# CSB5/XNA_Basecaller

Hardware: AMD Instinct MI355X
Metric: raw signal samples/sec basecalled, chunksize 10k (higher is better)
Workload: dtype f32 (feed-forward projections split-f16x3 MFMA, recurrent projections f16 MFMA + FP8 block-scaled correction MFMA, f32 accumulate; CRF decode f32)

## Files before the change

xna_basecaller_amd/csrc/xb_api.hip:

```cpp
#include <hip/hip_runtime.h>

#include <algorithm>
#include <cmath>
#include <cstdarg>
#include <cstdio>
#include <cstdlib>
#include <cstring>
#include <map>
#include <string>
#include <vector>

#include "../../include/xna_basecaller.h"
#include "xb_internal.h"

using xb::half_t;

namespace {

thread_local std::string g_create_error;

struct DevBuf {
    void *p = nullptr;
    size_t bytes = 0;
};
// ... 2230 lines not shown
    float *d_sig = reinterpret_cast<float *>(base);
    double *d_lev = reinterpret_cast<double *>(base + b_sig);
    double *d_win = reinterpret_cast<double *>(base + b_sig + b_lev), *d_cost = d_win + b_f64 / 8;
    int32_t *d_bp = reinterpret_cast<int32_t *>(base + b_sig + b_lev + 2 * b_f64);
    int8_t *d_ok = reinterpret_cast<int8_t *>(d_bp) + b_bp;
    XB_HIP(ctx, hipMemcpyAsync(d_sig, signal, C * N * 4, hipMemcpyHostToDevice, ctx->stream));
    XB_HIP(ctx, hipMemcpyAsync(d_lev, levels, total * 8, hipMemcpyHostToDevice, ctx->stream));
    if (band) XB_HIP(ctx, hipMemcpyAsync(d_win, window, C * 8, hipMemcpyHostToDevice, ctx->stream));
    if (int rc = dtw_run(ctx, d_sig, n, N, d_lev, offsets, ref_rep, d_win, band, Kmax, {d_bp, d_ok, d_cost})) return rc;
    XB_HIP(ctx, hipMemcpyAsync(breakpoints, d_bp, C * Kmax * 4, hipMemcpyDeviceToHost, ctx->stream));
    XB_HIP(ctx, hipMemcpyAsync(ok, d_ok, C, hipMemcpyDeviceToHost, ctx->stream));
    XB_HIP(ctx, hipMemcpyAsync(cost, d_cost, C * 8, hipMemcpyDeviceToHost, ctx->stream));
    return xb_synchronize(ctx);
}

XB_API int64_t xb_dtw_scratch_bytes(const xb_ctx *ctx) { return ctx ? (int64_t)ctx->dtw.scratch_written : 0; }

XB_API int xb_set_profiling(xb_ctx *ctx, int on)
{
    if (!ctx) return XB_ERR_INVALID;
    XB_HIP(ctx, hipSetDevice(ctx->device));
    if (int rc = flush_held(ctx)) return rc;
    ctx->profiling = on != 0;
    return XB_OK;
}

XB_API int xb_get_stage_times(xb_ctx *ctx, float ms[XB_STAGE_COUNT], int64_t launches[XB_STAGE_COUNT])
{
    if (!ctx) return XB_ERR_INVALID;
    XB_HIP(ctx, hipSetDevice(ctx->device));
    if (int rc = flush_held(ctx)) return rc;
    if (int rc = sync_all(ctx)) return rc;
    collect_events(ctx);
    for (int i = 0; i < XB_STAGE_COUNT; ++i) {
        if (ms) ms[i] = ctx->stage_ms[i];
        if (launches) launches[i] = ctx->stage_launches[i];
    }
    return XB_OK;
}

XB_API int xb_reset_stage_times(xb_ctx *ctx)
{
    if (!ctx) return XB_ERR_INVALID;
    if (int rc = flush_held(ctx)) return rc;
    if (int rc = sync_all(ctx)) return rc;
    collect_events(ctx);
    for (int i = 0; i < XB_STAGE_COUNT; ++i) { ctx->stage_ms[i] = 0.f; ctx->stage_launches[i] = 0; }
    return XB_OK;
}

XB_API int xb_geometry(const xb_ctx *ctx, int *T, int *S, int *C_blank, int *C_noblank)
{
    if (!ctx) return XB_ERR_INVALID;
    if (T) *T = ctx->T;
    if (S) *S = ctx->S;
    if (C_blank) *C_blank = ctx->S * (ctx->cfg.n_base + 1);
    if (C_noblank) *C_noblank = ctx->O;
    return XB_OK;
}

XB_API int xb_debug_layer_output(xb_ctx *ctx, int which, int n, uint16_t *hi, uint16_t *second)
{
    if (!ctx || !hi || !second || which < 0 || which > 1) return XB_ERR_INVALID;
    if (n < 1 || n > ctx->cap) return fail(ctx, XB_ERR_INVALID, "batch %d outside [1, %d]", n, ctx->cap);
    XB_HIP(ctx, hipSetDevice(ctx->device));
    if (int rc = join_async_decode(ctx)) return rc;
    if (int rc = sync_all(ctx)) return rc;
    const size_t bytes = sizeof(uint16_t) * (size_t)ctx->T * n * ctx->cfg.features;
    XB_HIP(ctx, hipMemcpy(hi, ctx->x_hi[which], bytes, hipMemcpyDeviceToHost));
    XB_HIP(ctx, hipMemcpy(second, ctx->x_lo[which], bytes, hipMemcpyDeviceToHost));
    return XB_OK;
}

#ifdef XB_LSTM_STAMPS
XB_API int xb_debug_lstm_stamps(xb_ctx *ctx, unsigned long long out[10], int reset)
{
    if (!ctx) return XB_ERR_INVALID;
    XB_HIP(ctx, hipStreamSynchronize(ctx->stream));
    xb::lstm_read_stamps(out, reset != 0);
    return XB_OK;
}
#endif
#ifdef XB_GEMM_STAMPS
XB_API int xb_debug_gemm_stamps(xb_ctx *ctx, unsigned long long out[8], int reset)
{
    if (!ctx) return XB_ERR_INVALID;
    if (int rc = sync_all(ctx)) return rc;
    xb::gemm_read_stamps(out, reset != 0);
    return XB_OK;
}
#endif

}
```

xna_basecaller_amd/csrc/xb_encoder.hip:

```cpp
#include "xb_enc_common.h"

namespace {

constexpr int CF_TT = 32;

__global__ __launch_bounds__(256) void conv_front_kernel(xb::ConvFrontParams p)
{
    extern __shared__ __attribute__((aligned(16))) unsigned char smem_raw[];
    const int tid = threadIdx.x;
    const int n = blockIdx.y;
    const int t0 = blockIdx.x * CF_TT;
    const int W = p.winlen, ST = p.stride, pad = W / 2, L = p.L;
    const int nq = (CF_TT - 1) * ST + W;
    const int q0 = t0 * ST - pad;
    float *sig = reinterpret_cast<float *>(smem_raw);
    float *a1 = sig + nq + 8;
    float *a2 = a1 + 4 * (nq + 4);
    float *w2s = a2 + 16 * nq;
    float *b2s = w2s + 320, *w1s = b2s + 16, *b1s = w1s + 20;

    for (int i = tid; i < 320; i += 256) w2s[i] = p.w2[i];
    if (tid < 16) b2s[tid] = p.b2[tid];
    if (tid < 20) w1s[tid] = p.w1[tid];
    if (tid < 4) b1s[tid] = p.b1[tid];
// ... 173 lines not shown
        return;
    }
    if (EPI == xb::EPI_TANH_SCALE && interior && !p.expand) {
        float *tile = p.out_f32 + (size_t)mw * p.ldc + nw;
        const int loff = (HS * (lane >> 5)) * p.ldc + (lane & 31);
#pragma unroll
        for (int i = 0; i < 4; ++i)
#pragma unroll
            for (int r = 0; r < 16; ++r) {
                float *rowp = tile + (size_t)(i * 32 + acc_row<L16>(r)) * p.ldc;
#pragma unroll
                for (int j = 0; j < 2; ++j) rowp[loff + j * 32] = p.scale * fast_tanh(acc[i][j][r] + bj[j]);
            }
        return;
    }
    if (EPI == xb::EPI_SILU_SPLIT && interior) {
        const size_t tile = (size_t)mw * p.ldc + nw;
        const int loff = (HS * (lane >> 5)) * p.ldc + (lane & 31);
        unsigned char *q8base = reinterpret_cast<unsigned char *>(p.out_lo) + tile * 2;
        const int qoff = (HS * (lane >> 5)) * p.ldc * 2 + (lane & 31);
#pragma unroll
        for (int i = 0; i < 4; ++i)
#pragma unroll
            for (int r = 0; r < 16; ++r) {
                const size_t ro = (size_t)(i * 32 + acc_row<L16>(r)) * p.ldc;
#pragma unroll
                for (int j = 0; j < 2; ++j) {
                    const float v = silu(acc[i][j][r] + bj[j]);
                    if (out_q8) {
                        half_t hi;
                        unsigned char h8, l8;
                        q8_bytes(v, p.out_exp, hi, h8, l8);
                        p.out_hi[tile + ro + loff + j * 32] = hi;
                        unsigned char *q = q8base + ro * 2 + qoff + j * 64;
                        q[0] = h8;
                        q[32] = l8;
                    } else {
                        half_t hi, lo;
                        split_f16(v, hi, lo);
                        p.out_hi[tile + ro + loff + j * 32] = hi;
                        p.out_lo[tile + ro + loff + j * 32] = lo;
                    }
                }
            }
        return;
    }
#pragma unroll
    for (int i = 0; i < 4; ++i)
#pragma unroll
        for (int j = 0; j < 2; ++j) {
            const int n = nw + j * 32 + (lane & 31);
            if (n >= p.Nn) continue;
            const float bias = bj[j];
            int ocol = n;
            if (EPI == xb::EPI_TANH_SCALE && p.expand) ocol = (n / p.nb) * (p.nb + 1) + 1 + n % p.nb;
#pragma unroll
            for (int r = 0; r < 16; ++r) {
                const int m = mw + i * 32 + acc_row<L16>(r) + HS * (lane >> 5);
                if (m >= p.M) continue;
                const float v = acc[i][j][r] + bias;
                if (EPI == xb::EPI_BIAS_F32) {
                    p.out_f32[p.gin_n ? xb::gin_offset((size_t)m, n, p.gin_n, p.Nn) : (size_t)m * p.ldc + n] = v;
                } else if (EPI == xb::EPI_SILU_SPLIT) {
                    if (out_q8) {
                        half_t hi;
                        unsigned char h8, l8;
                        q8_bytes(silu(v), p.out_exp, hi, h8, l8);
                        unsigned char *q = reinterpret_cast<unsigned char *>(p.out_lo) + q8_offset((size_t)m, p.ldc, n);
                        p.out_hi[(size_t)m * p.ldc + n] = hi;
                        q[0] = h8;
                        q[32] = l8;
                    } else {
                        half_t hi, lo;
                        split_f16(silu(v), hi, lo);
                        p.out_hi[(size_t)m * p.ldc + n] = hi;
                        p.out_lo[(size_t)m * p.ldc + n] = lo;
                    }
                } else {
                    p.out_f32[(size_t)m * p.ldc + ocol] = p.scale * fast_tanh(v);
                    if (p.expand && n % p.nb == 0) p.out_f32[(size_t)m * p.ldc + ocol - 1] = p.blank;
                }
            }
        }
}

#define G8_BARRIER()                                   \
    do {                                               \
        __builtin_amdgcn_sched_barrier(0);             \
        __builtin_amdgcn_s_barrier();                  \
        __builtin_amdgcn_sched_barrier(0);             \
    } while (0)

template <int EPI, int NSPLIT>
__global__ __launch_bounds__(GTHREADS) void gemm8r_kernel(xb::GemmParams p)
{
    constexpr int NP = NSPLIT == 1 ? 1 : 2;
    constexpr int PARTB = 128 * 64;
    constexpr int HTB = NP * PARTB;
    extern __shared__ __attribute__((aligned(16))) unsigned char smem_raw[];
    const int tid = threadIdx.x, lane = tid & 63;
    const int wid = __builtin_amdgcn_readfirstlane(tid >> 6);
    const int wr = wid >> 2, wc = wid & 3;
    int m0, n0;
    if (!gemm_tile_origin(p, m0, n0)) return;
    const int nk = p.K / GBK;

    unsigned offs[4];
    {
        const int drow = 16 * wid + (lane >> 2), dch = ((lane & 3) ^ ((lane >> 4) & 3)) * 8;
        const int Mrem = p.M - 1 - m0, Nrem = p.Nn - 1 - n0;
        int r;
        r = drow;        offs[0] = (unsigned)(((r > Mrem ? Mrem : r) * p.lda + dch) * 2);
        r = 128 + drow;  offs[1] = (unsigned)(((r > Mrem ? Mrem : r) * p.lda + dch) * 2);
        r = drow;        offs[2] = (unsigned)(((r > Nrem ? Nrem : r) * p.ldb + dch) * 2);
        r = 128 + drow;  offs[3] = (unsigned)(((r > Nrem ? Nrem : r) * p.ldb + dch) * 2);
    }
    const unsigned char *const tA_hi = reinterpret_cast<const unsigned char *>(p.a_hi + (size_t)m0 * p.lda);
    const unsigned char *const tA_lo = reinterpret_cast<const unsigned char *>(p.a_lo + (size_t)m0 * p.lda);
    const unsigned char *const tB_hi = reinterpret_cast<const unsigned char *>(p.b_hi + (size_t)n0 * p.ldb);
    const unsigned char *const tB_lo = reinterpret_cast<const unsigned char *>(p.b_lo + (size_t)n0 * p.ldb);
    unsigned char *const wdst = smem_raw + wid * 1024;
    u32x4 st[4][NP];
    unsigned char *const ldst = wdst + lane * 16;
#define G8_LOAD(h, t)                                                                           \
    do {                                                                                        \
        const size_t kb_ = (size_t)(t) * (GBK * 2);                                             \
        st[(h)][0] = *reinterpret_cast<const u32x4 *>(((h) < 2 ? tA_hi : tB_hi) + kb_ + offs[(h)]); \
        if (NP == 2) st[(h)][1] = *reinterpret_cast<const u32x4 *>(((h) < 2 ? tA_lo : tB_lo) + kb_ + offs[(h)]); \
    } while (0)
#define G8_WRITE(h, t)                                                                          \
    do {                                                                                        \
        unsigned char *dst_ = ldst + (((h) * 2 + ((t) & 1)) * HTB);                             \
        *reinterpret_cast<u32x4 *>(dst_) = st[(h)][0];                                          \
        if (NP == 2) *reinterpret_cast<u32x4 *>(dst_ + PARTB) = st[(h)][1];                     \
    } while (0)

    unsigned la[2];
#pragma unroll
    for (int ks = 0; ks < 2; ++ks)
        la[ks] = (unsigned)((lane & 31) * 64 + (((2 * ks + (lane >> 5)) ^ ((lane >> 2) & 3)) * 16));
    constexpr bool S16 = NSPLIT == 3;
    const unsigned la16 = (unsigned)((lane & 15) * 64 + (((lane >> 4) ^ ((lane >> 2) & 3)) * 16));
    const unsigned char *const fragA = smem_raw + wr * 2 * HTB;
    const unsigned char *const fragB = smem_raw + (2 + (wc >> 1)) * 2 * HTB + (wc & 1) * 4096;

    unsigned lqa[2], lqb[2];
#pragma unroll
    for (int j = 0; j < 2; ++j) {
        const int h = lane >> 5, sw = (lane >> 2) & 3;
        lqa[j] = (unsigned)((lane & 31) * 64 + (((2 * h + j) ^ sw) * 16));
        lqb[j] = (unsigned)((lane & 31) * 64 + (((2 * (1 - h) + j) ^ sw) * 16));
    }
    const int sca = 127 - p.a_exp - 11, scb = 127 - p.b_exp;

    half8 ah[2][2], al[2][2], bh[2], bl[2];
    v8i aq[2], bq;
#define G8_READ_A(d, mh)                                                                                  \
    _Pragma("unroll") for (int i2 = 0; i2 < 2; ++i2) {                                                    \
        const unsigned char *t_ = fragA + (d) * HTB + ((mh) * 2 + i2) * 2048;                         \
        _Pragma("unroll") for (int ks = 0; ks < 2; ++ks) {                                                \
            ah[i2][ks] = *reinterpret_cast<const half8 *>(t_ + (S16 ? ks * 1024 + la16 : la[ks]));        \
            if (S16) al[i2][ks] = *reinterpret_cast<const half8 *>(t_ + PARTB + ks * 1024 + la16);       \
        }                                                                                                 \
        if (NSPLIT == 2) {                                                                                \
            const v4i x_ = *reinterpret_cast<const v4i *>(t_ + PARTB + lqa[0]);                           \
            const v4i y_ = *reinterpret_cast<const v4i *>(t_ + PARTB + lqa[1]);                           \
// ... 45 lines not shown

    floatx16 acc[4][2];
    f32x4 acc16[8][4];
#pragma unroll
    for (int i = 0; i < 4; ++i)
#pragma unroll
        for (int j = 0; j < 2; ++j)
#pragma unroll
            for (int r = 0; r < 16; ++r) acc[i][j][r] = 0.0f;
#pragma unroll
    for (int i = 0; i < 8; ++i)
#pragma unroll
        for (int j = 0; j < 4; ++j)
#pragma unroll
            for (int r = 0; r < 4; ++r) acc16[i][j][r] = 0.0f;

#pragma unroll
    for (int h = 0; h < 4; ++h) G8_LOAD(h, 0);
#pragma unroll
    for (int h = 0; h < 4; ++h) G8_WRITE(h, 0);
#pragma unroll
    for (int h = 0; h < 4; ++h) G8_LOAD(h, nk > 1 ? 1 : 0);
    asm volatile("s_waitcnt lgkmcnt(0)" ::: "memory");
    G8_BARRIER();
    if (wr == 1) G8_BARRIER();

#define G8_MOVE(q, t)                                                                       \
    do {                                                                                    \
        G8_WRITE(q, (t) + 1);                                                               \
        __builtin_amdgcn_sched_barrier(0);       \
        G8_LOAD(q, (t) + 2 < nk ? (t) + 2 : nk - 1);                                        \
        asm volatile("s_waitcnt lgkmcnt(0)" ::: "memory");                                  \
    } while (0)
#define G8_TILE(d, t)                                                                       \
    do {                                                                                    \
        G8_READ_B(d, 0);                                                                    \
        G8_READ_A(d, 0);                                                                    \
        G8_MOVE(0, t);                                                                      \
        G8_BARRIER();                                                                       \
        G8_MFMA(0, 0);                                                                      \
        G8_BARRIER();                                                                       \
        G8_READ_B(d, 1);                                                                    \
        G8_MOVE(1, t);                                                                      \
        G8_BARRIER();                                                                       \
        G8_MFMA(0, 1);                                                                      \
        G8_BARRIER();                                                                       \
        G8_READ_A(d, 1);                                                                    \
        G8_MOVE(2, t);                                                                      \
        G8_BARRIER();                                                                       \
        G8_MFMA(1, 1);                                                                      \
        G8_BARRIER();                                                                       \
        G8_READ_B(d, 0);                                                                    \
        G8_MOVE(3, t);                                                                      \
        G8_BARRIER();                                                                       \
        G8_MFMA(1, 0);                                                                      \
        G8_BARRIER();                                                                       \
    } while (0)

    int t = 0;
    for (; t + 1 < nk; t += 2) {
        G8_TILE(0, t);
        G8_TILE(1, t + 1);
    }
    if (t < nk) G8_TILE(0, t);
    if (wr == 0) G8_BARRIER();
#undef G8_MOVE
#undef G8_LOAD
#undef G8_WRITE
#undef G8_TILE
#undef G8_MFMA
#undef G8_F16
#undef G8_S16
#undef G8_READ_A
#undef G8_READ_B

    int lane_e = lane, mw_e = m0 + wr * 128, nw_e = n0 + wc * 64;
    asm volatile("" : "+v"(lane_e), "+s"(mw_e), "+s"(nw_e));
    if constexpr (S16) acc16_lines(acc16, acc);
    gemm_epilogue<EPI, S16>(p, acc, mw_e, nw_e, lane_e);
}

constexpr int G4_BM = 128, G4_BN = 256, G4_THREADS = 256;
#ifdef XB_GEMM_STAMPS
__device__ unsigned long long g_gemm_stamps[8];
#define G4P_STAMP(i) do { const unsigned long long n_ = __builtin_readcyclecounter(); st_acc[(i)] += n_ - st_prev; st_prev = n_; } while (0)
#else
#define G4P_STAMP(i) do { } while (0)
#endif

__device__ __forceinline__ bool gemm4_tile_origin(const xb::GemmParams &p, int &m0, int &n0)
{
    const int MT = (p.M + G4_BM - 1) / G4_BM, NT = (p.Nn + G4_BN - 1) / G4_BN;
    const int snw = p.sn > 0 ? p.sn : gemm_super_n(NT);
    const int SN = NT < snw ? NT : snw, SM = 64 / SN;
    const int ngroups = (NT + SN - 1) / SN, msup = (MT + SM - 1) / SM;
    const int b = blockIdx.x, xcd = b & 7, j = b >> 3;
    const int q = (j >> 6) * 8 + xcd, w = j & 63;
    if (q >= msup * ngroups || w >= SM * SN) return false;
    const int mt = (q / ngroups) * SM + w / SN, nt = (q % ngroups) * SN + w % SN;
    if (mt >= MT || nt >= NT) return false;
    m0 = mt * G4_BM;
    n0 = nt * G4_BN;
    return true;
}

template <int EPI, int NSPLIT>
__global__ __launch_bounds__(G4_THREADS, 2) void gemm4p_kernel(xb::GemmParams p)
{
    constexpr int NPA = NSPLIT == 1 ? 1 : 2;
    constexpr int NPC = NSPLIT == 1 ? 2 : 4;
    constexpr int PARTB = 128 * 64;
    constexpr int STB = NPA * PARTB;
    constexpr int NA = 2 * NPA, NB = 2 * NPC;
    constexpr int INFL = 2 * NB + 2 * NA;
    extern __shared__ __attribute__((aligned(16))) unsigned char smem_raw[];
    const int tid = threadIdx.x, lane = tid & 63;
    const int wid = __builtin_amdgcn_readfirstlane(tid >> 6);
    int m0, n0;
    if (!gemm4_tile_origin(p, m0, n0)) return;
    const int nk = p.K / GBK;
#ifdef XB_GEMM_STAMPS
    unsigned long long st_prev = __builtin_readcyclecounter(), st_acc[5] = {0, 0, 0, 0, 0};
#endif

    unsigned offs[2];
    {
        const int r0 = tid >> 2, sc = ((tid & 3) ^ ((tid >> 4) & 3)) * 16;
        const int Mrem = p.M - 1 - m0;
        offs[0] = (unsigned)((r0 > Mrem ? Mrem : r0) * p.lda * 2 + sc);
        offs[1] = (unsigned)((r0 + 64 > Mrem ? Mrem : r0 + 64) * p.lda * 2 + sc);
    }
    const unsigned char *const tA_hi = reinterpret_cast<const unsigned char *>(p.a_hi + (size_t)m0 * p.lda);
    const unsigned char *const tA_lo = reinterpret_cast<const unsigned char *>(p.a_lo + (size_t)m0 * p.lda);
    auto dma_a = [&](int t, int stage, bool live = true) {
        const size_t kb = (size_t)t * (GBK * 2);
        unsigned char *dst = smem_raw + stage * STB + wid * 1024;
        const unsigned ol[2] = {live ? offs[0] : 0u, live ? offs[1] : 0u};
#pragma unroll
        for (int part = 0; part < NPA; ++part)
#pragma unroll
            for (int h = 0; h < 2; ++h) {
                const unsigned m0v = __builtin_amdgcn_readfirstlane(
                    (unsigned)(uintptr_t)(__attribute__((address_space(3))) void *)(dst + part * PARTB + h * 4096));
                asm volatile("s_mov_b32 m0, %2\n\ts_nop 0\n\tglobal_load_lds_dwordx4 %0, %1"
                             ::"v"(ol[h]), "s"((part ? tA_lo : tA_hi) + kb), "s"(m0v) : "memory", "m0");
            }
    };

    const unsigned boff = (unsigned)__builtin_amdgcn_readfirstlane((int)(((unsigned)(n0 + wid * 64) >> 5) * NPC * 1024u));
    const unsigned char *const tB = p.b4 + boff;
    const size_t bks = p.b4_kstride;
    const unsigned voff0 = (unsigned)lane * 16;
    u32x4 bE[2][NPC], bO[2][NPC];
#define G4P_LDB(dst, vo, base, j, pc)                                                           \
    asm volatile("global_load_dwordx4 %0, %1, %2 offset:%3" : "=v"(dst) : "v"(vo), "s"((base) + (j) * (NPC * 1024)), "i"((pc) * 1024))
#define G4P_LDB_GROUP_V(bS, vo, base, pc)                                                       \
    do {                                                                                        \
        G4P_LDB(bS[0][(pc)], vo, base, 0, pc);                                                  \
        G4P_LDB(bS[1][(pc)], vo, base, 1, pc);                                                  \
    } while (0)
#define G4P_LDB_GROUP(bS, base, pc) G4P_LDB_GROUP_V(bS, voff0, base, pc)
#define G4P_WAIT2(n, a, b) asm volatile("s_waitcnt vmcnt(%2)" : "+v"(a), "+v"(b) : "i"(n))
#define G4P_WAIT4(n, a, b, c, d) asm volatile("s_waitcnt vmcnt(%4)" : "+v"(a), "+v"(b), "+v"(c), "+v"(d) : "i"(n))

    const int hs = lane >> 5, sw = (lane >> 2) & 3;
    unsigned la[2], lqa[2];
#pragma unroll
    for (int j = 0; j < 2; ++j) {
        la[j] = (unsigned)((lane & 31) * 64 + (((2 * j + hs) ^ sw) * 16));
        lqa[j] = (unsigned)((lane & 31) * 64 + (((2 * hs + j) ^ sw) * 16));
    }
    const int sca = 127 - p.a_exp - 11, scb = 127 - p.b_exp;
    constexpr bool S16 = NSPLIT == 3;
    const unsigned la16 = (unsigned)((lane & 15) * 64 + (((lane >> 4) ^ sw) * 16));

    half8 xh[2], xl[2];
    floatx16 acc[4][2];
    f32x4 acc16[8][4];
#pragma unroll
    for (int i = 0; i < 4; ++i)
#pragma unroll
        for (int j = 0; j < 2; ++j)
#pragma unroll
            for (int r = 0; r < 16; ++r) acc[i][j][r] = 0.0f;
#pragma unroll
    for (int i = 0; i < 8; ++i)
#pragma unroll
        for (int j = 0; j < 4; ++j)
#pragma unroll
            for (int r = 0; r < 4; ++r) acc16[i][j][r] = 0.0f;

#define G4P_SB() __builtin_amdgcn_sched_barrier(0)
#define G4P_RD_H(d, sa, part, ih, ks)                                                           \
    _Pragma("unroll") for (int i_ = 0; i_ < 2; ++i_)                                            \
        d[i_] = *reinterpret_cast<const half8 *>((sa) + (part) * PARTB + ((ih) * 2 + i_) * 2048 + la[(ks)])
#define G4P_RD_Q(d, sa, ih)                                                                     \
    _Pragma("unroll") for (int i_ = 0; i_ < 2; ++i_) {                                          \
        const v4i x_ = *reinterpret_cast<const v4i *>((sa) + PARTB + ((ih) * 2 + i_) * 2048 + lqa[0]); \
        const v4i y_ = *reinterpret_cast<const v4i *>((sa) + PARTB + ((ih) * 2 + i_) * 2048 + lqa[1]); \
        d[i_] = __builtin_shufflevector(x_, y_, 0, 1, 2, 3, 4, 5, 6, 7);                        \
    }
#define G4P_F16(A_, ih, bS, pc)                                                                 \
    _Pragma("unroll") for (int i_ = 0; i_ < 2; ++i_)                                            \
        _Pragma("unroll") for (int j_ = 0; j_ < 2; ++j_)                                        \
            acc[(ih) * 2 + i_][j_] = __builtin_amdgcn_mfma_f32_32x32x16_f16(A_[i_], __builtin_bit_cast(half8, bS[j_][(pc)]), \
// ... 127 lines not shown
            G4P_LDB_GROUP_V(bS, vb_, b2, 0);                                                    \
            G4P_LDB_GROUP_V(bS, vb_, b2, 1);                                                    \
        } else {                                                                                \
             \
             \
             \
             \
            half8 ah0[2], ah1[2];                                                               \
            G4P_RD_H(ah0, sa, 0, 0, 0);                                                         \
            G4P_RD_H(ah1, sa, 0, 1, 0);                                                         \
            _Pragma("unroll") for (int ks = 0; ks < 2; ++ks) {                                  \
                 \
                 \
                constexpr int LA_ = NA;                                                         \
                if (ks == 0) G4P_WAIT2(INFL - 2 - LA_, bS[0][0], bS[1][0]);                     \
                else G4P_WAIT2(INFL - 2, bS[0][1], bS[1][1]);                                   \
                G4P_MFMA_BEGIN();                                                               \
                G4P_F16(ah0, 0, bS, ks);                                                        \
                G4P_MFMA_END();                                                                 \
                if (ks == 0) {                                                                  \
                    dma_a(t2_, nxt2, live_);                                                    \
                    G4P_RD_H(ah0, sa, 0, 0, 1);                                                 \
                }                                                                               \
                G4P_MFMA_BEGIN();                                                               \
                G4P_F16(ah1, 1, bS, ks);                                                        \
                G4P_MFMA_END();                                                                 \
                if (ks == 0) {                                                                  \
                    G4P_RD_H(ah1, sa, 0, 1, 1);                                                 \
                    G4P_LDB_GROUP_V(bS, vb_, b2, 0);                                            \
                } else {                                                                        \
                    G4P_LDB_GROUP_V(bS, vb_, b2, 1);                                            \
                }                                                                               \
            }                                                                                   \
        }                                                                                       \
        if constexpr (!S16) asm volatile("s_waitcnt lgkmcnt(0)" ::: "memory");                  \
        G4P_STAMP(3);                                                                           \
        { const int c_ = cur; cur = nxt1; nxt1 = nxt2; nxt2 = c_; }                             \
    } while (0)

    if (__builtin_amdgcn_readfirstlane(n0 + wid * 64 >= p.Nn ? 1 : 0)) {
        dma_a(0, 0);
        dma_a(nk > 1 ? 1 : 0, 1);
        int c0 = 0, c1 = 1, c2 = 2;
#pragma unroll 1
        for (int t = 0; t < nk + (S16 ? 1 : 0); ++t) {
            asm volatile("s_waitcnt vmcnt(%0)" ::"i"(NA) : "memory");
            __builtin_amdgcn_s_barrier();
            dma_a(t + 2 < nk ? t + 2 : nk - 1, c2, t + 2 < nk);
            const int c_ = c0; c0 = c1; c1 = c2; c2 = c_;
        }
        asm volatile("s_waitcnt vmcnt(0)" ::: "memory");
        return;
    }

    int cur = 0, nxt1 = 1, nxt2 = 2;
    {
        const int t1 = nk > 1 ? 1 : 0;
        const unsigned char *const b0 = tB, *const b1 = tB + (size_t)t1 * bks;
        dma_a(0, 0);
        if constexpr (NSPLIT == 2) {
            G4P_LDB_GROUP(bE, b0, 0); G4P_LDB_GROUP(bE, b0, 2); G4P_LDB_GROUP(bE, b0, 3); G4P_LDB_GROUP(bE, b0, 1);
        } else if constexpr (S16) {
            G4P_LDB_GROUP(bE, b0, 2); G4P_LDB_GROUP(bE, b0, 3); G4P_LDB_GROUP(bE, b0, 0); G4P_LDB_GROUP(bE, b0, 1);
        } else {
            G4P_LDB_GROUP(bE, b0, 0); G4P_LDB_GROUP(bE, b0, 1);
        }
        dma_a(t1, 1);
        if constexpr (NSPLIT == 2) {
            G4P_LDB_GROUP(bO, b1, 0); G4P_LDB_GROUP(bO, b1, 2); G4P_LDB_GROUP(bO, b1, 3); G4P_LDB_GROUP(bO, b1, 1);
        } else if constexpr (S16) {
            G4P_LDB_GROUP(bO, b1, 2); G4P_LDB_GROUP(bO, b1, 3); G4P_LDB_GROUP(bO, b1, 0); G4P_LDB_GROUP(bO, b1, 1);
        } else {
            G4P_LDB_GROUP(bO, b1, 0); G4P_LDB_GROUP(bO, b1, 1);
        }
    }
    if constexpr (S16) {
        asm volatile("s_waitcnt vmcnt(%0)" ::"i"(2 * NB + NA) : "memory");
        G4P_SB();
        __builtin_amdgcn_s_barrier();
        G4P_SB();
        G4P_RD16(xl, smem_raw, 1, 0);
        G4P_RD16(xh, smem_raw, 0, 0);
    }
    int t = 0;
#pragma unroll 1
    for (; t + 1 < nk; t += 2) {
        G4P_TILE(bE, t);
        G4P_TILE(bO, t + 1);
    }
    if (t < nk) G4P_TILE(bE, t);
    if constexpr (NSPLIT == 1)
        asm volatile("s_waitcnt vmcnt(0)" : "+v"(bE[0][0]), "+v"(bE[1][0]), "+v"(bE[0][1]), "+v"(bE[1][1]),
                       "+v"(bO[0][0]), "+v"(bO[1][0]), "+v"(bO[0][1]), "+v"(bO[1][1]) :: "memory");
    else
        asm volatile("s_waitcnt vmcnt(0)" : "+v"(bE[0][0]), "+v"(bE[1][0]), "+v"(bE[0][1]), "+v"(bE[1][1]),
                       "+v"(bE[0][2]), "+v"(bE[1][2]), "+v"(bE[0][3]), "+v"(bE[1][3]),
                       "+v"(bO[0][0]), "+v"(bO[1][0]), "+v"(bO[0][1]), "+v"(bO[1][1]),
                       "+v"(bO[0][2]), "+v"(bO[1][2]), "+v"(bO[0][3]), "+v"(bO[1][3]) :: "memory");
    G4P_SB();
#undef G4P_TILE
#undef G4P_LDB
#undef G4P_LDB_GROUP
#undef G4P_LDB_GROUP_V
#undef G4P_WAIT2
#undef G4P_WAIT4
#undef G4P_RD_H
#undef G4P_RD16
#undef G4P_M16
#undef G4P_S16
#undef G4P_WAIT8
#undef G4P_RD_Q
#undef G4P_F16
#undef G4P_F8
#undef G4P_MFMA_BEGIN
#undef G4P_MFMA_END
#undef G4P_SB

    int lane_e = lane, mw_e = m0, nw_e = n0 + wid * 64;
    asm volatile("" : "+v"(lane_e), "+s"(mw_e), "+s"(nw_e));
    if constexpr (S16) acc16_lines(acc16, acc);
    gemm_epilogue<EPI, S16>(p, acc, mw_e, nw_e, lane_e);
#ifdef XB_GEMM_STAMPS
    if (NSPLIT == 3) {
        asm volatile("s_waitcnt vmcnt(0)" ::: "memory");
        G4P_STAMP(4);
        if (tid == 0) {
            for (int i = 0; i < 5; ++i) atomicAdd(&g_gemm_stamps[i], st_acc[i]);
            atomicAdd(&g_gemm_stamps[5], (unsigned long long)(__builtin_amdgcn_s_getreg(4 | (0 << 6) | (3 << 11)) & 1u));
            atomicAdd(&g_gemm_stamps[6], 1ull);
            atomicAdd(&g_gemm_stamps[7], (unsigned long long)nk);
        }
    }
#endif
}

template <int EPI, int NSPLIT>
hipError_t launch_gemm_ns(const xb::GemmParams &p, hipStream_t stream)
{
    const int MT = (p.M + GBM - 1) / GBM, NT = (p.Nn + GBN - 1) / GBN;
    const int SN = gemm_super_n(NT), SM = 32 / SN;
    const int supers = ((NT + SN - 1) / SN) * ((MT + SM - 1) / SM);
    dim3 grid(8 * 32 * ((supers + 7) / 8)), block(GTHREADS);
    const size_t lds = (size_t)2 * 4 * (NSPLIT == 1 ? 1 : 2) * 128 * 64;
    (void)hipFuncSetAttribute(reinterpret_cast<const void *>(&gemm8r_kernel<EPI, NSPLIT>),
                              hipFuncAttributeMaxDynamicSharedMemorySize, (int)lds);
    hipLaunchKernelGGL((gemm8r_kernel<EPI, NSPLIT>), grid, block, lds, stream, p);
    return hipGetLastError();
}

template <int EPI, int NSPLIT>
hipError_t launch_gemm4p_ns(const xb::GemmParams &p, hipStream_t stream)
{
    const int MT = (p.M + G4_BM - 1) / G4_BM, NT = (p.Nn + G4_BN - 1) / G4_BN;
    const int snw = p.sn > 0 ? p.sn : gemm_super_n(NT);
    const int SN = NT < snw ? NT : snw, SM = 64 / SN;
    const int supers = ((NT + SN - 1) / SN) * ((MT + SM - 1) / SM);
    dim3 grid(8 * 64 * ((supers + 7) / 8)), block(G4_THREADS);
    size_t lds = (size_t)3 * (NSPLIT == 1 ? 1 : 2) * 128 * 64;
    if (p.one_per_cu) {
        lds = 96 * 1024;
        (void)hipFuncSetAttribute(reinterpret_cast<const void *>(&gemm4p_kernel<EPI, NSPLIT>),
                                  hipFuncAttributeMaxDynamicSharedMemorySize, (int)lds);
    }
    hipLaunchKernelGGL((gemm4p_kernel<EPI, NSPLIT>), grid, block, lds, stream, p);
    return hipGetLastError();
}

template <int EPI>
hipError_t launch_gemm_epi(const xb::GemmParams &p, hipStream_t stream)
{
    if (p.b4) {
        switch (p.nsplit) {
        case 1: return launch_gemm4p_ns<EPI, 1>(p, stream);
        case 2: return launch_gemm4p_ns<EPI, 2>(p, stream);
        default: return launch_gemm4p_ns<EPI, 3>(p, stream);
        }
    }
    switch (p.nsplit) {
    case 1: return launch_gemm_ns<EPI, 1>(p, stream);
    case 2: return launch_gemm_ns<EPI, 2>(p, stream);
    default: return launch_gemm_ns<EPI, 3>(p, stream);
    }
}

}


namespace xb {

#ifdef XB_GEMM_STAMPS
void gemm_read_stamps(unsigned long long out[8], bool reset)
{
    hipMemcpyFromSymbol(out, HIP_SYMBOL(g_gemm_stamps), sizeof(unsigned long long) * 8);
    if (reset) {
        unsigned long long z[8] = {};
        hipMemcpyToSymbol(HIP_SYMBOL(g_gemm_stamps), z, sizeof z);
    }
}
#endif

hipError_t launch_conv_front(const ConvFrontParams &p, hipStream_t stream)
{
    if (p.N < 1 || p.T < 1 || p.kp < 16 * p.winlen || p.kp % 32 != 0) return hipErrorInvalidValue;
    const int nq = (CF_TT - 1) * p.stride + p.winlen;
    const size_t lds = sizeof(float) * ((size_t)(nq + 8) + 4 * (nq + 4) + 16 * (size_t)nq + 360);
    if (lds > 60000) return hipErrorInvalidValue;
    dim3 grid((p.T + CF_TT - 1) / CF_TT, p.N), block(256);
    hipLaunchKernelGGL(conv_front_kernel, grid, block, lds, stream, p);
    return hipGetLastError();
}

hipError_t launch_gemm(const GemmParams &p, int epilogue, hipStream_t stream)
{
    if (p.M < 1 || p.Nn < 1 || p.K < GBK || p.K % GBK != 0 || p.lda % 8 != 0 || p.ldb % 8 != 0 ||
        p.lda < p.K || p.ldb < p.K)
        return hipErrorInvalidValue;
    if (p.nsplit < 1 || p.nsplit > 3) return hipErrorInvalidValue;
    switch (epilogue) {
    case EPI_BIAS_F32: return launch_gemm_epi<EPI_BIAS_F32>(p, stream);
    case EPI_SILU_SPLIT: return launch_gemm_epi<EPI_SILU_SPLIT>(p, stream);
    case EPI_TANH_SCALE: return launch_gemm_epi<EPI_TANH_SCALE>(p, stream);
    default: return hipErrorInvalidValue;
    }
}

}
```

xna_basecaller_amd/csrc/xb_internal.h:

```cpp
#pragma once
#include <hip/hip_runtime.h>
#include <stdint.h>

namespace xb {

typedef _Float16 half_t;

struct DecodeParams {
    const float *scores;
    int T, N, S, hi, nb;
    int cin, ld, has_blank;
    float blank;
    float *alpha, *beta, *bmax;
    float *qbuf;
    int ldq;
    float *logz;
    int stop_after;
    float *beta_out;
    int post_mode;
    int8_t *labels;
    int8_t *seq;
    int32_t *seq_len;
    char alphabet[8];
    int debug_stop;
// ... 116 lines not shown
    int spread;
    int dual;
    int slab;
    int xcd_local;
    unsigned *sig_flag;
    unsigned *sig_done;
    unsigned sig_base;
    int sig_nts;
};
hipError_t launch_lstm(const LstmParams &p, hipStream_t stream);
int lstm_resident_per_cu(int F, int nsplit, int dual);
int lstm_members(int F);
int lstm_group_chunks();
bool lstm_supported_features(int F);
constexpr int MAP_MAX_TEMPLATE = 4096;
constexpr int MAP_MAX_ROW = 4096;
constexpr int MAP_CHUNK_BYTES = 16384;
constexpr int MAP_PARTIAL_INTS = 6;
struct MapParams {
    const int8_t *seq;
    const int32_t *seq_len;
    int n, W;
    const uint8_t *tcodes;
    const int32_t *toff;
    const int32_t *chunk_first;
    int R, Lmax, nchunks;
    int match, mismatch, gap_open, gap_extend, ambiguous;
    int32_t *partial;
    int32_t *tmpl, *score, *second, *q_st, *q_en, *r_st, *r_en, *n_ops;
    int8_t *strand;
    uint8_t *ops;
    uint8_t *scratch;
    int trace_wgs;
};
inline int map_cols_per_lane(int Lmax) { return Lmax <= 64 ? 1 : (Lmax <= 128 ? 2 : 4); }
bool map_trace_in_lds(int W, int Lmax);
hipError_t launch_map_score(const MapParams &p, hipStream_t stream);
hipError_t launch_map_trace(const MapParams &p, hipStream_t stream);

constexpr int CTC_FAILED_SEQ = 1, CTC_FAILED_MAP = 2, CTC_SKIPPED_NON_UB = 4, CTC_FAILED_ACC = 8, CTC_FAILED_COV = 16;
inline int ctc_target_width(int Lmax) { return (Lmax + 15) & ~15; }
struct CtcTargetParams {
    const int32_t *seq_len;
    int n, W, cap;
    const int32_t *tmpl, *q_st, *q_en, *r_st, *r_en, *n_ops;
    const int8_t *strand;
    const uint8_t *ops;
    const uint8_t *tcodes;
    const int32_t *toff;
    int R, TW;
    double min_accuracy, min_coverage;
    int ub_only, ub_plus, ub_minus;
    int32_t *mlen, *blen, *target_len;
    uint8_t *verdict;
    uint8_t *target;
};
hipError_t launch_ctc_targets(const CtcTargetParams &p, hipStream_t stream);

constexpr int DTW_MAX_SAMPLES = 65535;
constexpr int DTW_MAX_COLUMNS = 65535;
struct DtwParams {
    const float *signal;
    const double *levels;
    const int32_t *off;
    const double *window;
    int N, rep, Kmax;
    int first, count;
    unsigned long long *scratch;
    size_t choice_words, slot_words;
    int32_t *bp;
    int8_t *ok;
    double *cost;
};
inline int dtw_cols_per_lane(int Mmax) { return Mmax <= 64 ? 1 : (Mmax <= 128 ? 2 : 4); }
constexpr size_t dtw_stripe_words(int N, int M, int cols) { return (size_t)((N - M + 64 * cols + 63) & ~63) * cols; }
constexpr size_t dtw_choice_words(int N, int M, int cols)
{
    return M > N ? 0 : (size_t)((M + 64 * cols - 1) / (64 * cols)) * dtw_stripe_words(N, M, cols);
}
hipError_t launch_dtw(const DtwParams &p, int cols, bool band, hipStream_t stream);

#ifdef XB_LSTM_STAMPS
void lstm_read_stamps(unsigned long long out[10], bool reset);
void gemm_read_stamps(unsigned long long out[8], bool reset);
#endif

}
```

Before: 43.45 million.

## Peel last K tile of split-f16x3 GEMM and interleave fp32 epilogue stores with MFMAs

New measurement: 43.92 million (median of 6 runs). 1.1% higher.

```diff
diff --git a/xna_basecaller_amd/csrc/xb_api.hip b/xna_basecaller_amd/csrc/xb_api.hip
--- a/xna_basecaller_amd/csrc/xb_api.hip
+++ b/xna_basecaller_amd/csrc/xb_api.hip
@@ -2336,7 +2336,7 @@
 }
 #endif
 #ifdef XB_GEMM_STAMPS
-XB_API int xb_debug_gemm_stamps(xb_ctx *ctx, unsigned long long out[8], int reset)
+XB_API int xb_debug_gemm_stamps(xb_ctx *ctx, unsigned long long out[12], int reset)
 {
     if (!ctx) return XB_ERR_INVALID;
     if (int rc = sync_all(ctx)) return rc;
diff --git a/xna_basecaller_amd/csrc/xb_encoder.hip b/xna_basecaller_amd/csrc/xb_encoder.hip
--- a/xna_basecaller_amd/csrc/xb_encoder.hip
+++ b/xna_basecaller_amd/csrc/xb_encoder.hip
@@ -279,6 +279,44 @@
                 }
             }
         }
+}
+
+template <int EPI>
+struct EpiRows {
+    float *tile;
+    int ld, loff;
+    float bj[2];
+};
+
+template <int EPI, bool L16>
+__device__ __forceinline__ void epi_rows_init(const xb::GemmParams &p, int mw, int nw, int lane, EpiRows<EPI> &e)
+{
+    static_assert(EPI == xb::EPI_BIAS_F32, "fp32 rows only");
+    e.ld = p.ldc;
+    e.tile = p.out_f32 + (size_t)mw * p.ldc + nw;
+    if (p.gin_n) {
+        const int n = p.gin_n, t0 = mw / n, c0 = mw - t0 * n;
+        e.ld = 128;
+        e.tile = p.out_f32 + (((size_t)t0 * (p.Nn >> 7) + (size_t)(nw >> 7)) * n + c0) * 128 + (nw & 127);
+    }
+    e.loff = ((L16 ? 8 : 4) * (lane >> 5)) * e.ld + (lane & 31);
+}
+
+template <int EPI>
+__device__ __forceinline__ void epi_rows_bias(const xb::GemmParams &p, int nw, int lane, EpiRows<EPI> &e)
+{
+    e.bj[0] = e.bj[1] = 0.0f;
+    if (p.bias) {
+        e.bj[0] = p.bias[nw + (lane & 31)];
+        e.bj[1] = p.bias[nw + 32 + (lane & 31)];
+    }
+}
+
+template <int EPI, bool L16>
+__device__ __forceinline__ void epi_rows_store(const EpiRows<EPI> &e, int i, int j, int r, float a)
+{
+    float *q = e.tile + (size_t)(i * 32 + acc_row<L16>(r)) * e.ld + e.loff + j * 32;
+    __builtin_nontemporal_store(a + e.bj[j], q);
 }
 
 #define G8_BARRIER()                                   \
@@ -490,10 +528,26 @@
 
 constexpr int G4_BM = 128, G4_BN = 256, G4_THREADS = 256;
 #ifdef XB_GEMM_STAMPS
-__device__ unsigned long long g_gemm_stamps[8];
+__device__ unsigned long long g_gemm_stamps[12];
 #define G4P_STAMP(i) do { const unsigned long long n_ = __builtin_readcyclecounter(); st_acc[(i)] += n_ - st_prev; st_prev = n_; } while (0)
+#define G4P_FLUSH_STAMPS(nkt)                                                                   \
+    do {                                                                                        \
+        if (NSPLIT == 3) {                                                                      \
+            G4P_STAMP(6);                                                                       \
+            asm volatile("s_waitcnt vmcnt(0)" ::: "memory");                                    \
+            G4P_STAMP(7);                                                                       \
+            if (tid == 0) {                                                                     \
+                for (int i = 0; i < 5; ++i) atomicAdd(&g_gemm_stamps[i], st_acc[i]);            \
+                for (int i = 5; i < 9; ++i) atomicAdd(&g_gemm_stamps[3 + i], st_acc[i]);        \
+                atomicAdd(&g_gemm_stamps[5], (unsigned long long)(__builtin_amdgcn_s_getreg(4 | (0 << 6) | (3 << 11)) & 1u)); \
+                atomicAdd(&g_gemm_stamps[6], 1ull);                                             \
+                atomicAdd(&g_gemm_stamps[7], (unsigned long long)(nkt));                        \
+            }                                                                                   \
+        }                                                                                       \
+    } while (0)
 #else
 #define G4P_STAMP(i) do { } while (0)
+#define G4P_FLUSH_STAMPS(nkt) do { } while (0)
 #endif
 
 __device__ __forceinline__ bool gemm4_tile_origin(const xb::GemmParams &p, int &m0, int &n0)
@@ -512,8 +566,8 @@
     return true;
 }
 
-template <int EPI, int NSPLIT>
-__global__ __launch_bounds__(G4_THREADS, 2) void gemm4p_kernel(xb::GemmParams p)
+template <int EPI, int NSPLIT, bool PEEL>
+__device__ __forceinline__ void gemm4p_body(const xb::GemmParams &p)
 {
     constexpr int NPA = NSPLIT == 1 ? 1 : 2;
     constexpr int NPC = NSPLIT == 1 ? 2 : 4;
@@ -528,7 +582,7 @@
     if (!gemm4_tile_origin(p, m0, n0)) return;
     const int nk = p.K / GBK;
 #ifdef XB_GEMM_STAMPS
-    unsigned long long st_prev = __builtin_readcyclecounter(), st_acc[5] = {0, 0, 0, 0, 0};
+    unsigned long long st_prev = __builtin_readcyclecounter(), st_acc[9] = {0, 0, 0, 0, 0, 0, 0, 0, 0};
 #endif
 
     unsigned offs[2];
@@ -822,23 +876,120 @@
         G4P_RD16(xl, smem_raw, 1, 0);
         G4P_RD16(xh, smem_raw, 0, 0);
     }
+#define G4P_EPI_UNIT(i, ib, jp)                                                                 \
+    do {                                                                                        \
+        _Pragma("unroll") for (int r_ = 0; r_ < 4; ++r_) {                                      \
+            float u_ = acc16[2 * (i) + (ib)][2 * (jp)][r_], v_ = acc16[2 * (i) + (ib)][2 * (jp) + 1][r_]; \
+            asm volatile("v_permlane16_swap_b32 %0, %1" : "+v"(u_), "+v"(v_));                  \
+            epi_rows_store<EPI, true>(er, (i), (jp), (ib) * 8 + r_, u_);                        \
+            epi_rows_store<EPI, true>(er, (i), (jp), (ib) * 8 + 4 + r_, v_);                    \
+        }                                                                                       \
+        G4P_SB();                                                                               \
+    } while (0)
+     \
+#define G4P_LAST_PHASE(AH_, AL_, q, bS)                                                         \
+    do {                                                                                        \
+        G4P_MFMA_BEGIN();                                                                       \
+        G4P_M16(AL_, q, bS, 0);                                                                 \
+        G4P_MFMA_END();                                                                         \
+        G4P_EPI_UNIT((q) - 1, 0, 0);                                                            \
+        G4P_MFMA_BEGIN();                                                                       \
+        G4P_M16(AH_, q, bS, 2);                                                                 \
+        G4P_MFMA_END();                                                                         \
+        G4P_EPI_UNIT((q) - 1, 0, 1);                                                            \
+        G4P_MFMA_BEGIN();                                                                       \
+        G4P_M16(AH_, q, bS, 0);                                                                 \
+        G4P_MFMA_END();                                                                         \
+    } while (0)
+#define G4P_LAST(bS, bX)                                                                        \
+    do {                                                                                        \
+        const unsigned char *const sa = smem_raw + cur * STB;                                   \
+        half8 yh[2], yl[2];                                                                     \
+        G4P_RD16(yl, sa, 1, 1);                                                                 \
+        G4P_RD16(yh, sa, 0, 1);                                                                 \
+        G4P_WAIT8(NB + NA, bS);                                                                 \
+        G4P_SB();                                                                               \
+        epi_rows_bias<EPI>(p, n0 + wid * 64, lane, er);                                         \
+        G4P_MFMA_BEGIN();                                                                       \
+        G4P_S16(xh, xl, 0, bS);                                                                 \
+        G4P_MFMA_END();                                                                         \
+        G4P_RD16(xl, sa, 1, 2);                                                                 \
+        G4P_RD16(xh, sa, 0, 2);                                                                 \
+        G4P_WAIT8(0, bX);                                                                       \
+        G4P_SB();                                                                               \
+        G4P_LAST_PHASE(yh, yl, 1, bS);                                                          \
+        G4P_RD16(yl, sa, 1, 3);                                                                 \
+        G4P_RD16(yh, sa, 0, 3);                                                                 \
+        G4P_EPI_UNIT(0, 1, 0);                                                                  \
+        G4P_EPI_UNIT(0, 1, 1);                                                                  \
+        G4P_LAST_PHASE(xh, xl, 2, bS);                                                          \
+        G4P_EPI_UNIT(1, 1, 0);                                                                  \
+        G4P_EPI_UNIT(1, 1, 1);                                                                  \
+        asm volatile("s_waitcnt lgkmcnt(0)" ::: "memory");                                      \
+        G4P_SB();                                                                               \
+        __builtin_amdgcn_s_barrier();                                                           \
+        G4P_SB();                                                                               \
+        G4P_LAST_PHASE(yh, yl, 3, bS);                                                          \
+        G4P_EPI_UNIT(2, 1, 0);                                                                  \
+        G4P_EPI_UNIT(2, 1, 1);                                                                  \
+        G4P_STAMP(8);                                                                           \
+         \
+         \
+        asm volatile("s_nop 7\n\ts_nop 7");                                                     \
+        G4P_EPI_UNIT(3, 0, 0);                                                                  \
+        G4P_EPI_UNIT(3, 0, 1);                                                                  \
+        G4P_EPI_UNIT(3, 1, 0);                                                                  \
+        G4P_EPI_UNIT(3, 1, 1);                                                                  \
+    } while (0)
+
+#define G4P_FINISH()                                                                            \
+    do {                                                                                        \
+        if constexpr (NSPLIT == 1)                                                              \
+            asm volatile("s_waitcnt vmcnt(0)" : "+v"(bE[0][0]), "+v"(bE[1][0]), "+v"(bE[0][1]), "+v"(bE[1][1]), \
+                           "+v"(bO[0][0]), "+v"(bO[1][0]), "+v"(bO[0][1]), "+v"(bO[1][1]) :: "memory"); \
+        else                                                                                    \
+            asm volatile("s_waitcnt vmcnt(0)" : "+v"(bE[0][0]), "+v"(bE[1][0]), "+v"(bE[0][1]), "+v"(bE[1][1]), \
+                           "+v"(bE[0][2]), "+v"(bE[1][2]), "+v"(bE[0][3]), "+v"(bE[1][3]),      \
+                           "+v"(bO[0][0]), "+v"(bO[1][0]), "+v"(bO[0][1]), "+v"(bO[1][1]),      \
+                           "+v"(bO[0][2]), "+v"(bO[1][2]), "+v"(bO[0][3]), "+v"(bO[1][3]) :: "memory"); \
+        G4P_SB();                                                                               \
+        int lane_e = lane, mw_e = m0, nw_e = n0 + wid * 64;                                     \
+        asm volatile("" : "+v"(lane_e), "+s"(mw_e), "+s"(nw_e));                                \
+        G4P_STAMP(4);                                                                           \
+        if constexpr (S16) acc16_lines(acc16, acc);                                             \
+        G4P_STAMP(5);                                                                           \
+        gemm_epilogue<EPI, S16>(p, acc, mw_e, nw_e, lane_e);                                    \
+        G4P_FLUSH_STAMPS(nk);                                                                   \
+    } while (0)
+
     int t = 0;
+    if constexpr (PEEL) {
+        static_assert(S16 && EPI == xb::EPI_BIAS_F32, "the peeled tile: three products, gin / plain fp32 rows");
 #pragma unroll 1
-    for (; t + 1 < nk; t += 2) {
+        for (; t + 2 < nk; t += 2) {
+            G4P_TILE(bE, t);
+            G4P_TILE(bO, t + 1);
+        }
         G4P_TILE(bE, t);
-        G4P_TILE(bO, t + 1);
-    }
-    if (t < nk) G4P_TILE(bE, t);
-    if constexpr (NSPLIT == 1)
-        asm volatile("s_waitcnt vmcnt(0)" : "+v"(bE[0][0]), "+v"(bE[1][0]), "+v"(bE[0][1]), "+v"(bE[1][1]),
-                       "+v"(bO[0][0]), "+v"(bO[1][0]), "+v"(bO[0][1]), "+v"(bO[1][1]) :: "memory");
-    else
-        asm volatile("s_waitcnt vmcnt(0)" : "+v"(bE[0][0]), "+v"(bE[1][0]), "+v"(bE[0][1]), "+v"(bE[1][1]),
-                       "+v"(bE[0][2]), "+v"(bE[1][2]), "+v"(bE[0][3]), "+v"(bE[1][3]),
-                       "+v"(bO[0][0]), "+v"(bO[1][0]), "+v"(bO[0][1]), "+v"(bO[1][1]),
-                       "+v"(bO[0][2]), "+v"(bO[1][2]), "+v"(bO[0][3]), "+v"(bO[1][3]) :: "memory");
-    G4P_SB();
+        EpiRows<EPI> er;
+        epi_rows_init<EPI, true>(p, m0, n0 + wid * 64, lane, er);
+        G4P_LAST(bO, bE);
+        G4P_FLUSH_STAMPS(nk - 1);
+        return;
+    } else {
+#pragma unroll 1
+        for (; t + 1 < nk; t += 2) {
+            G4P_TILE(bE, t);
+            G4P_TILE(bO, t + 1);
+        }
+        if (t < nk) G4P_TILE(bE, t);
+    }
+    G4P_FINISH();
+#undef G4P_FINISH
 #undef G4P_TILE
+#undef G4P_LAST
+#undef G4P_LAST_PHASE
+#undef G4P_EPI_UNIT
 #undef G4P_LDB
 #undef G4P_LDB_GROUP
 #undef G4P_LDB_GROUP_V
@@ -855,23 +1006,22 @@
 #undef G4P_MFMA_BEGIN
 #undef G4P_MFMA_END
 #undef G4P_SB
-
-    int lane_e = lane, mw_e = m0, nw_e = n0 + wid * 64;
-    asm volatile("" : "+v"(lane_e), "+s"(mw_e), "+s"(nw_e));
-    if constexpr (S16) acc16_lines(acc16, acc);
-    gemm_epilogue<EPI, S16>(p, acc, mw_e, nw_e, lane_e);
-#ifdef XB_GEMM_STAMPS
-    if (NSPLIT == 3) {
-        asm volatile("s_waitcnt vmcnt(0)" ::: "memory");
-        G4P_STAMP(4);
-        if (tid == 0) {
-            for (int i = 0; i < 5; ++i) atomicAdd(&g_gemm_stamps[i], st_acc[i]);
-            atomicAdd(&g_gemm_stamps[5], (unsigned long long)(__builtin_amdgcn_s_getreg(4 | (0 << 6) | (3 << 11)) & 1u));
-            atomicAdd(&g_gemm_stamps[6], 1ull);
-            atomicAdd(&g_gemm_stamps[7], (unsigned long long)nk);
-        }
-    }
-#endif
+}
+
+inline bool gemm_peel_ok(const xb::GemmParams &p)
+{
+    return p.M % G4_BM == 0 && p.Nn % G4_BN == 0 && p.K >= 2 * GBK && p.K % (2 * GBK) == 0 && p.gin_n % 128 == 0;
+}
+
+template <int EPI, int NSPLIT>
+__global__ __launch_bounds__(G4_THREADS, 2) void gemm4p_kernel(xb::GemmParams p)
+{
+    gemm4p_body<EPI, NSPLIT, false>(p);
+}
+
+__global__ __launch_bounds__(G4_THREADS, 2) void gemm4p_peel_kernel(xb::GemmParams p)
+{
+    gemm4p_body<xb::EPI_BIAS_F32, 3, true>(p);
 }
 
 template <int EPI, int NSPLIT>
@@ -897,12 +1047,15 @@
     const int supers = ((NT + SN - 1) / SN) * ((MT + SM - 1) / SM);
     dim3 grid(8 * 64 * ((supers + 7) / 8)), block(G4_THREADS);
     size_t lds = (size_t)3 * (NSPLIT == 1 ? 1 : 2) * 128 * 64;
+    const bool peel = EPI == xb::EPI_BIAS_F32 && NSPLIT == 3 && gemm_peel_ok(p);
+    const void *const fn = peel ? reinterpret_cast<const void *>(&gemm4p_peel_kernel)
+                                : reinterpret_cast<const void *>(&gemm4p_kernel<EPI, NSPLIT>);
     if (p.one_per_cu) {
         lds = 96 * 1024;
-        (void)hipFuncSetAttribute(reinterpret_cast<const void *>(&gemm4p_kernel<EPI, NSPLIT>),
-                                  hipFuncAttributeMaxDynamicSharedMemorySize, (int)lds);
-    }
-    hipLaunchKernelGGL((gemm4p_kernel<EPI, NSPLIT>), grid, block, lds, stream, p);
+        (void)hipFuncSetAttribute(fn, hipFuncAttributeMaxDynamicSharedMemorySize, (int)lds);
+    }
+    if (peel) hipLaunchKernelGGL(gemm4p_peel_kernel, grid, block, lds, stream, p);
+    else hipLaunchKernelGGL((gemm4p_kernel<EPI, NSPLIT>), grid, block, lds, stream, p);
     return hipGetLastError();
 }
 
@@ -929,11 +1082,11 @@
 namespace xb {
 
 #ifdef XB_GEMM_STAMPS
-void gemm_read_stamps(unsigned long long out[8], bool reset)
-{
-    hipMemcpyFromSymbol(out, HIP_SYMBOL(g_gemm_stamps), sizeof(unsigned long long) * 8);
+void gemm_read_stamps(unsigned long long out[12], bool reset)
+{
+    hipMemcpyFromSymbol(out, HIP_SYMBOL(g_gemm_stamps), sizeof(unsigned long long) * 12);
     if (reset) {
-        unsigned long long z[8] = {};
+        unsigned long long z[12] = {};
         hipMemcpyToSymbol(HIP_SYMBOL(g_gemm_stamps), z, sizeof z);
     }
 }
diff --git a/xna_basecaller_amd/csrc/xb_internal.h b/xna_basecaller_amd/csrc/xb_internal.h
--- a/xna_basecaller_amd/csrc/xb_internal.h
+++ b/xna_basecaller_amd/csrc/xb_internal.h
@@ -222,7 +222,7 @@
 
 #ifdef XB_LSTM_STAMPS
 void lstm_read_stamps(unsigned long long out[10], bool reset);
-void gemm_read_stamps(unsigned long long out[8], bool reset);
+void gemm_read_stamps(unsigned long long out[12], bool reset);
 #endif
 
 }
```
